# DillionLowry/NeuralCodecs

Hardware: AMD Instinct MI355X
Metric: audio-seconds/sec encode+decode (x real-time), DAC-44.1kHz B=32 (higher is better)
Workload: dtype f32; 1 GPU; DAC 44.1kHz 8kbps encode+decode, batch=32 x 1 s clips per GPU (BASELINE configs[1]); clips_per_gpu=32, global_batch=32, collective=none

## Files before the change

neuralcodecs_amd/csrc/nc_chunk.hip:

```cpp
#include <algorithm>

#include "nc_limits.h"
#include "nc_model.h"

namespace nc {

namespace {

int64_t ceil_div(int64_t a, int64_t b) { return (a + b - 1) / b; }
int64_t round_up(int64_t a, int64_t m) { return ceil_div(a, m) * m; }

void halo_from_layers(const int32_t* er, int ne, const int32_t* dr, int nd, int final_reach, int W, int vq_max, int64_t align, nc_halo* out) {
    if (ne <= 0 || ne > 8 || nd <= 0 || nd > 8) fail(NC_EINVAL, "encoder/decoder rate lists must hold 1..8 entries");
    int64_t l = final_reach, r = final_reach, hop = 1;
    if (W > 1) { l += W - 1; r += W - 1; }
    for (int i = ne - 1; i >= 0; --i) {
        const int64_t s = er[i], p = (s + 1) / 2;
        if (s <= 0) fail(NC_EINVAL, "encoder rate must be positive");
        l = l * s + p; r = r * s + (2 * s - 1 - p);
        l += 39; r += 39;
        hop *= s;
    }
    l += 3; r += 3;
    int64_t a = 3, b = 3, H = 1;
// ... 47 lines not shown
    if (setting < 0) return P;
    int64_t chunk = 0;
    if (setting > 0) chunk = round_up(setting, h.align);
    else if (!fits) chunk = auto_chunk(h, kind == CK_DECODE);
    if (chunk <= 0 || frames <= chunk) return P;
    P.chunk = chunk;
    P.n_chunks = ceil_div(frames, chunk);
    if (kind == CK_ENCODE) { P.halo_l = h.enc_right; P.halo_r = h.enc_left; }
    if (kind == CK_DECODE) { P.halo_l = h.dec_right; P.halo_r = h.dec_left; }
    return P;
}

struct Window { int64_t f0, f1, w0, w1; };
Window window_of(const ChunkPlan& P, int64_t j, int64_t frames) {
    Window w;
    w.f0 = j * P.chunk; w.f1 = std::min(frames, w.f0 + P.chunk);
    w.w0 = std::max<int64_t>(0, w.f0 - P.halo_l); w.w1 = std::min(frames, w.f1 + P.halo_r);
    return w;
}
int64_t max_window(const ChunkPlan& P, int64_t frames) { return std::min(frames, P.chunk + P.halo_l + P.halo_r); }

}

void Codec::copy2d(void* dst, bool dst_host, size_t dpitch, const void* src, bool src_host, size_t spitch, size_t width, size_t rows) {
    if (!width || !rows) return;
    if (!dst_host && !src_host) { launch_copy_rows(dst, dpitch, src, spitch, width, rows, stream); return; }
    const hipMemcpyKind kind = dst_host ? (src_host ? hipMemcpyHostToHost : hipMemcpyDeviceToHost) : hipMemcpyHostToDevice;
    if (rows == 1 || (width == dpitch && width == spitch)) NC_HIP(hipMemcpyAsync(dst, src, width * rows, kind, stream));
    else NC_HIP(hipMemcpy2DAsync(dst, dpitch, src, spitch, width, rows, kind, stream));
}

static void dac_halo(const nc_dac_config& c, nc_halo* out) {
    halo_from_layers(c.encoder_rates, c.n_encoder_rates, c.decoder_rates, c.n_decoder_rates, 1, 0, 1, 1, out);
}

ChunkPlan DacModel::chunk_plan(ChunkKind kind, int B, int64_t Tz) const {
    if (B <= 0 || Tz <= 0) fail(NC_EINVAL, "B and frames must be positive");
    nc_halo h{};
    dac_halo(cfg, &h);
    const bool fits = chunk_frames != 0 || oneshot_fits(cfg.encoder_rates, cfg.n_encoder_rates, cfg.encoder_dim, cfg.decoder_rates,
                                                        cfg.n_decoder_rates, cfg.decoder_dim, kind, Tz);
    ChunkPlan P = make_plan(chunk_frames, h, kind, Tz, fits);
    const int64_t W = P.n_chunks > 1 ? max_window(P, Tz) : Tz;
    int64_t maxel = 0;
    if (kind == CK_ENCODE) {
        int c = cfg.encoder_dim;
        int64_t L = W * hop;
        maxel = (int64_t)c * pitch16(L);
        for (int i = 0; i < cfg.n_encoder_rates; ++i) { c *= 2; L /= cfg.encoder_rates[i]; maxel = std::max(maxel, (int64_t)c * pitch16(L)); }
    } else if (kind == CK_DECODE) {
        int64_t L = W;
        maxel = (int64_t)cfg.decoder_dim * pitch16(L);
        for (int i = 0; i < cfg.n_decoder_rates; ++i) { L *= cfg.decoder_rates[i]; maxel = std::max(maxel, (int64_t)(cfg.decoder_dim >> (i + 1)) * pitch16(L)); }
    }
    P.arena_bytes = 3 * (int64_t)B * maxel * 4;
    return P;
}

void DacModel::encode_chunked(const ChunkPlan& P, bool host, const float* pcm, int B, int64_t T, int sample_rate, int n_q, int64_t* codes, float* z,
                              float* latents, int64_t* codes_tq) {
    if (!pcm || !(codes || codes_tq)) fail(NC_EINVAL, "pcm and codes must not be null");
    if (B <= 0 || T <= 0) fail(NC_EINVAL, "B and T must be positive");
    if (T > (int64_t)1 << 30) fail(NC_EINVAL, "clip too long");
    use_device();
    const int nq = codes_tq ? cfg.n_codebooks : ((n_q <= 0 || n_q > cfg.n_codebooks) ? cfg.n_codebooks : n_q);
    const int D = cfg.codebook_dim;
    const int64_t Tz = frames(T);
    for (int64_t j = 0; j < P.n_chunks; ++j) {
        const Window w = window_of(P, j, Tz);
        const int64_t s0 = w.w0 * hop, Tw = std::min(T, w.w1 * hop) - s0, Wf = w.w1 - w.w0, k0 = w.f0 - w.w0, n = w.f1 - w.f0;
        ck_in.reserve((size_t)B * Tw * 4);
        ck_codes.reserve((size_t)B * nq * Wf * 8);
        copy2d(ck_in.p, false, (size_t)Tw * 4, pcm + s0, host, (size_t)T * 4, (size_t)Tw * 4, (size_t)B);
        if (codes_tq) {
            encode_code_matrix_dev(ck_in.as<float>(), B, Tw, sample_rate, ck_codes.as<int64_t>());
            copy2d(codes_tq + w.f0 * nq, host, (size_t)Tz * nq * 8, ck_codes.as<int64_t>() + k0 * nq, false, (size_t)Wf * nq * 8, (size_t)n * nq * 8, (size_t)B);
            continue;
        }
        if (z) ck_a.reserve((size_t)B * latent * Wf * 4);
        if (latents) ck_b.reserve((size_t)B * nq * D * Wf * 4);
        encode_dev(ck_in.as<float>(), B, Tw, sample_rate, n_q, ck_codes.as<int64_t>(), z ? ck_a.as<float>() : nullptr, latents ? ck_b.as<float>() : nullptr);
        copy2d(codes + w.f0, host, (size_t)Tz * 8, ck_codes.as<int64_t>() + k0, false, (size_t)Wf * 8, (size_t)n * 8, (size_t)B * nq);
        if (z) copy2d(z + w.f0, host, (size_t)Tz * 4, ck_a.as<float>() + k0, false, (size_t)Wf * 4, (size_t)n * 4, (size_t)B * latent);
        if (latents) copy2d(latents + w.f0, host, (size_t)Tz * 4, ck_b.as<float>() + k0, false, (size_t)Wf * 4, (size_t)n * 4, (size_t)B * nq * D);
    }
}

void DacModel::from_codes_chunked(const ChunkPlan& P, bool host, const int64_t* codes, int B, int n_q, int64_t Tz, float* z) {
    if (!codes || !z) fail(NC_EINVAL, "codes and z must not be null");
    if (B <= 0 || Tz <= 0 || n_q <= 0 || n_q > cfg.n_codebooks) fail(NC_EINVAL, "bad codes shape [%d,%d,%lld]", B, n_q, (long long)Tz);
    use_device();
    for (int64_t j = 0; j < P.n_chunks; ++j) {
        const Window w = window_of(P, j, Tz);
        const int64_t n = w.f1 - w.f0;
        ck_codes.reserve((size_t)B * n_q * n * 8);
        ck_a.reserve((size_t)B * latent * n * 4);
        copy2d(ck_codes.p, false, (size_t)n * 8, codes + w.f0, host, (size_t)Tz * 8, (size_t)n * 8, (size_t)B * n_q);
        from_codes_dev(ck_codes.as<int64_t>(), B, n_q, n, ck_a.as<float>());
        copy2d(z + w.f0, host, (size_t)Tz * 4, ck_a.p, false, (size_t)n * 4, (size_t)n * 4, (size_t)B * latent);
    }
}

void DacModel::decode_chunked(const ChunkPlan& P, bool host, const float* z, const int64_t* codes_tq, int n_q, int B, int64_t Tz, float* pcm) {
    if (!(z || codes_tq) || !pcm) fail(NC_EINVAL, "z and pcm must not be null");
    if (B <= 0 || Tz <= 0) fail(NC_EINVAL, "B and frames must be positive");
    if (codes_tq && (n_q <= 0 || n_q > cfg.n_codebooks)) fail(NC_EINVAL, "bad code matrix shape [%d,%lld,%d]", B, (long long)Tz, n_q);
    use_device();
    int64_t H = 1;
    for (int i = 0; i < cfg.n_decoder_rates; ++i) H *= cfg.decoder_rates[i];
    const int64_t Lfull = decoded_len(Tz);
    for (int64_t j = 0; j < P.n_chunks; ++j) {
        const Window w = window_of(P, j, Tz);
        const int64_t Wf = w.w1 - w.w0, Lw = decoded_len(Wf), o0 = w.f0 * H, o1 = w.f1 == Tz ? Lfull : w.f1 * H, k0 = (w.f0 - w.w0) * H;
        if (o1 <= o0) continue;
        if (k0 + (o1 - o0) > Lw) fail(NC_ESTATE, "internal: decoded window of %lld samples does not cover its chunk", (long long)Lw);
        ck_out.reserve((size_t)B * Lw * 4);
        if (codes_tq) {
            ck_codes.reserve((size_t)B * Wf * n_q * 8);
            copy2d(ck_codes.p, false, (size_t)Wf * n_q * 8, codes_tq + w.w0 * n_q, host, (size_t)Tz * n_q * 8, (size_t)Wf * n_q * 8, (size_t)B);
            decode_code_matrix_dev(ck_codes.as<int64_t>(), B, Wf, n_q, ck_out.as<float>());
        } else {
            ck_a.reserve((size_t)B * latent * Wf * 4);
            copy2d(ck_a.p, false, (size_t)Wf * 4, z + w.w0, host, (size_t)Tz * 4, (size_t)Wf * 4, (size_t)B * latent);
            decode_dev(ck_a.as<float>(), B, Wf, ck_out.as<float>());
        }
        copy2d(pcm + o0, host, (size_t)Lfull * 4, ck_out.as<float>() + k0, false, (size_t)Lw * 4, (size_t)(o1 - o0) * 4, (size_t)B);
    }
}

static void snac_halo(const nc_snac_config& c, nc_halo* out) {
    if (c.n_vq_strides <= 0 || c.n_vq_strides > 8) fail(NC_EINVAL, "vq stride list must hold 1..8 entries");
    const int W = c.attn_window_size > 0 ? c.attn_window_size : 1;
    int64_t a = c.vq_strides[0], x = a, y = W;
    if (a <= 0) fail(NC_EINVAL, "vq stride must be positive");
    while (y) { const int64_t t = x % y; x = y; y = t; }
    const int64_t align = a / x * W;
    int vq_max = 1;
// ... 182 lines not shown
```

neuralcodecs_amd/csrc/nc_dac.hip:

```cpp
#include <cstdlib>
#include <cstring>

#include "nc_model.h"

namespace nc {

Codec::~Codec() {
    if (own_stream) (void)hipStreamDestroy(own_stream);
}

void Codec::init_device(int device_index) {
    int n = 0;
    if (hipGetDeviceCount(&n) != hipSuccess || n <= 0) fail(NC_EDEVICE, "no HIP device available (the engine has no CPU fallback)");
    if (device_index < 0 || device_index >= n) fail(NC_EINVAL, "device index %d out of range (0..%d)", device_index, n - 1);
    device = device_index;
    NC_HIP(hipSetDevice(device));
    hipDeviceProp_t prop;
    NC_HIP(hipGetDeviceProperties(&prop, device));
    if (std::strncmp(prop.gcnArchName, "gfx950", 6) != 0)
        fail(NC_EDEVICE, "device %d is %s; this engine is built for gfx950 (MI355X) only", device, prop.gcnArchName);
    cu_count = prop.multiProcessorCount;
    lds_per_cu = prop.maxSharedMemoryPerMultiProcessor;
    NC_HIP(hipStreamCreateWithFlags(&own_stream, hipStreamNonBlocking));
    stream = own_stream;
}

void Codec::use_device() const { NC_HIP(hipSetDevice(device)); }

void Codec::switch_stream(hipStream_t s) {
    if (s == stream) return;
    use_device();
    hipEvent_t e;
// ... 143 lines not shown
        load_alpha(b, p + ".block.0.alpha", in_dim, dec[bi].a_up);
        load_wn_conv(b, p + ".block.1", dec[bi].up, in_dim, out_dim, 2 * s, s, (s + 1) / 2, 1, true, NC_KC_CONV_UP);
        for (int u = 0; u < 3; ++u) {
            snprintf(nm, sizeof nm, "decoder.model.%d.block.%d", bi + 1, u + 2);
            const std::string q = nm;
            load_alpha(b, q + ".block.0.alpha", out_dim, dec[bi].ru[u].a1);
            load_wn_conv(b, q + ".block.1", dec[bi].ru[u].c7, out_dim, out_dim, 7, 1, 3 * kDil[u], kDil[u], false, NC_KC_CONV_K7);
            load_alpha(b, q + ".block.2.alpha", out_dim, dec[bi].ru[u].a2);
            load_wn_conv(b, q + ".block.3", dec[bi].ru[u].c1, out_dim, out_dim, 1, 1, 0, 1, false, NC_KC_CONV_K1);
        }
    }
    snprintf(nm, sizeof nm, "decoder.model.%d.alpha", cfg.n_decoder_rates + 1);
    load_alpha(b, nm, out_dim, dec_alpha_out);
    snprintf(nm, sizeof nm, "decoder.model.%d", cfg.n_decoder_rates + 2);
    load_wn_conv(b, nm, dec_out, out_dim, 1, 7, 1, 3, 1, false, NC_KC_HEAD);
    NC_HIP(hipDeviceSynchronize());
    loaded = true;
}

int64_t DacModel::decoded_len(int64_t fr) const {
    int64_t L = fr;
    for (int i = 0; i < cfg.n_decoder_rates; ++i) {
        const int s = cfg.decoder_rates[i];
        L = (L - 1) * s - 2 * ((s + 1) / 2) + 2 * s;
    }
    return L;
}

static int64_t row_pitch(int64_t L) {
    static const bool on = env_flag("NC_DAC_PITCH");
    return (on && L >= 256) ? ((L + 15) & ~(int64_t)15) : L;
}

float* DacModel::run_res_unit(ResUnit& ru, int dil, float* cur, int C, int64_t L, int B, int& cur_idx, const float* alpha_next) {
    (void)dil;
    const int64_t P = row_pitch(L);
    const int h_idx = (cur_idx + 1) % 3, o_idx = (cur_idx + 2) % 3;
    float* h = act[h_idx].as<float>();
    float* o = act[o_idx].as<float>();
    ConvIO io{};
    io.x = cur; io.x_bstride = (int64_t)C * P; io.x_cstride = P; io.x_len = (int32_t)L; io.Tin = L;
    io.alpha_in = ru.a1.as<float>(); io.alpha_out = ru.a2.as<float>();
    static const bool wide_192 = env_flag("NC_WIDE_FUSE_192");
    if (fuse_res_units && can_fuse_res_unit(ru.c7, ru.c1) && (C != 192 || wide_192)) {
        io.res = cur; io.fuse_k1 = &ru.c1; io.alpha_out2 = alpha_next;
        io.y = o; io.y_bstride = (int64_t)C * P; io.y_cstride = P;
        launch_conv(ru.c7, io, B, stream, &prof);
        cur_idx = o_idx;
        return o;
    }
    io.y = h; io.y_bstride = (int64_t)C * P; io.y_cstride = P;
    launch_conv(ru.c7, io, B, stream, &prof);
    ConvIO i2{};
    i2.x = h; i2.x_bstride = (int64_t)C * P; i2.x_cstride = P; i2.x_len = (int32_t)L; i2.Tin = L;
    i2.res = cur; i2.alpha_out = alpha_next;
    i2.y = o; i2.y_bstride = (int64_t)C * P; i2.y_cstride = P;
    launch_conv(ru.c1, i2, B, stream, &prof);
    cur_idx = o_idx;
    return o;
}

void DacModel::encode_dev(const float* pcm, int B, int64_t T, int sample_rate, int n_q, int64_t* codes, float* z, float* latents) {
    if (!loaded) fail(NC_ESTATE, "weights not loaded (call nc_codec_load_weights first)");
    if (!pcm || !codes) fail(NC_EINVAL, "pcm and codes must not be null");
    if (B <= 0 || T <= 0) fail(NC_EINVAL, "B and T must be positive");
    if (sample_rate != 0 && sample_rate != cfg.sample_rate)
        fail(NC_EINVAL, "Input audio sample rate %dHz does not match model sample rate %dHz", sample_rate, cfg.sample_rate);
    if (T > (int64_t)1 << 30) fail(NC_EINVAL, "clip too long");
    use_device();
    const int nq = (n_q <= 0 || n_q > cfg.n_codebooks) ? cfg.n_codebooks : n_q;
    const int64_t Tp = padded_len(T), Tz = frames(T);
    int64_t maxel = 0;
    {
        int c = cfg.encoder_dim;
        int64_t L = Tp;
        maxel = (int64_t)c * row_pitch(L);
        for (int i = 0; i < cfg.n_encoder_rates; ++i) {
            c *= 2;
            L /= cfg.encoder_rates[i];
            if ((int64_t)c * row_pitch(L) > maxel) maxel = (int64_t)c * row_pitch(L);
        }
    }
    for (auto& a : act) a.reserve((size_t)B * maxel * sizeof(float));
    const int D = cfg.codebook_dim;
    resid.reserve((size_t)B * latent * Tz * 4);
    zq.reserve((size_t)B * latent * Tz * 4);
    lat.reserve((size_t)B * nq * D * Tz * 4);
    st.reserve((size_t)B * D * Tz * 4);

    int C = cfg.encoder_dim;
    int64_t L = Tp;
    int cur_idx = 0;
    float* cur = act[0].as<float>();
    {
        ConvIO io{};
        io.x = pcm; io.x_bstride = T; io.x_cstride = T; io.x_len = (int32_t)T; io.Tin = Tp;
        io.y = cur; io.y_bstride = (int64_t)C * row_pitch(L); io.y_cstride = row_pitch(L);
        launch_conv(enc_stem, io, B, stream, &prof);
    }
    for (int bi = 0; bi < cfg.n_encoder_rates; ++bi) {
        for (int u = 0; u < 3; ++u)
            cur = run_res_unit(enc[bi].ru[u], kDil[u], cur, C, L, B, cur_idx, u == 2 ? enc[bi].a_down.as<float>() : nullptr);
        const int s = cfg.encoder_rates[bi];
        const int64_t Lo = enc[bi].down.out_len(L);
        const int o_idx = (cur_idx + 1) % 3;
        float* o = act[o_idx].as<float>();
        ConvIO io{};
        io.x = cur; io.x_bstride = (int64_t)C * row_pitch(L); io.x_cstride = row_pitch(L); io.x_len = (int32_t)L; io.Tin = L;
        if (bi + 1 == cfg.n_encoder_rates) io.alpha_out = enc_alpha_out.as<float>();
        io.y = o; io.y_bstride = (int64_t)2 * C * row_pitch(Lo); io.y_cstride = row_pitch(Lo);
        launch_conv(enc[bi].down, io, B, stream, &prof);
        (void)s;
        cur = o; cur_idx = o_idx; C *= 2; L = Lo;
    }
    if (L != Tz) fail(NC_ESTATE, "internal: encoder produced %lld frames, expected %lld", (long long)L, (long long)Tz);
    float* residual = resid.as<float>();
    {
        ConvIO io{};
        io.x = cur; io.x_bstride = (int64_t)C * row_pitch(L); io.x_cstride = row_pitch(L); io.x_len = (int32_t)L; io.Tin = L;
        io.y = residual; io.y_bstride = (int64_t)latent * Tz; io.y_cstride = Tz;
        launch_conv(enc_out, io, B, stream, &prof);
    }
    float* zq_d = z ? z : zq.as<float>();
    float* lat_d = latents ? latents : lat.as<float>();
    if (launch_dac_rvq_fused(rvq_stages.as<RvqStage>(), nq, latent, D, cfg.codebook_size, residual, B, Tz, codes, zq_d, lat_d, stream, &prof)) return;
    NC_HIP(hipMemsetAsync(zq_d, 0, (size_t)B * latent * Tz * 4, stream));
    for (int i = 0; i < nq; ++i) {
        ConvIO pi{};
        pi.x = residual; pi.x_bstride = (int64_t)latent * Tz; pi.x_cstride = Tz; pi.x_len = (int32_t)Tz; pi.Tin = Tz;
        pi.y = lat_d + (int64_t)i * D * Tz; pi.y_bstride = (int64_t)nq * D * Tz; pi.y_cstride = Tz;
        launch_conv(*in_proj[i], pi, B, stream, &prof);
        launch_vq_argmin(*codebooks[i], lat_d + (int64_t)i * D * Tz, (int64_t)nq * D * Tz, B, Tz, codes + (int64_t)i * Tz,
                         (int64_t)nq * Tz, st.as<float>(), stream, &prof);
        ConvIO po{};
        po.x = st.as<float>(); po.x_bstride = (int64_t)D * Tz; po.x_cstride = Tz; po.x_len = (int32_t)Tz; po.Tin = Tz;
        po.y = zq_d; po.y_bstride = (int64_t)latent * Tz; po.y_cstride = Tz;
        po.rvq_zq = zq_d; po.rvq_res = residual; po.epi = EPI_RVQ;
        launch_conv(*out_proj[i], po, B, stream, &prof);
    }
}

void DacModel::from_codes_dev(const int64_t* codes, int B, int n_q, int64_t Tz, float* z) {
    if (!loaded) fail(NC_ESTATE, "weights not loaded (call nc_codec_load_weights first)");
    if (!codes || !z) fail(NC_EINVAL, "codes and z must not be null");
    if (B <= 0 || Tz <= 0 || n_q <= 0 || n_q > cfg.n_codebooks) fail(NC_EINVAL, "bad codes shape [%d,%d,%lld]", B, n_q, (long long)Tz);
    use_device();
    const int D = cfg.codebook_dim;
    st.reserve((size_t)B * D * Tz * 4);
    NC_HIP(hipMemsetAsync(z, 0, (size_t)B * latent * Tz * 4, stream));
    for (int i = 0; i < n_q; ++i) {
        launch_vq_gather(*codebooks[i], codes + (int64_t)i * Tz, (int64_t)n_q * Tz, B, Tz, st.as<float>(), stream, &prof);
        ConvIO po{};
        po.x = st.as<float>(); po.x_bstride = (int64_t)D * Tz; po.x_cstride = Tz; po.x_len = (int32_t)Tz; po.Tin = Tz;
        po.y = z; po.y_bstride = (int64_t)latent * Tz; po.y_cstride = Tz;
        po.rvq_zq = z; po.rvq_res = nullptr; po.epi = EPI_RVQ;
        launch_conv(*out_proj[i], po, B, stream, &prof);
    }
}

__global__ void code_matrix_transpose_kernel(const int64_t* __restrict__ src, int64_t* __restrict__ dst, int B, int R, int C) {
    const int64_t i = (int64_t)blockIdx.x * 256 + threadIdx.x;
    if (i >= (int64_t)B * R * C) return;
    const int64_t c = i % C, r = (i / C) % R, b = i / ((int64_t)R * C);
    dst[(b * C + c) * R + r] = src[i];
}

void DacModel::decode_code_matrix_dev(const int64_t* codes_tq, int B, int64_t Tz, int n_q, float* pcm) {
    if (!codes_tq || !pcm) fail(NC_EINVAL, "codes and pcm must not be null");
    if (B <= 0 || Tz <= 0 || n_q <= 0 || n_q > cfg.n_codebooks) fail(NC_EINVAL, "bad code matrix shape [%d,%lld,%d]", B, (long long)Tz, n_q);
    use_device();
    codes_ws.reserve((size_t)B * n_q * Tz * 8);
    zq.reserve((size_t)B * latent * Tz * 4);
    const int64_t n = (int64_t)B * Tz * n_q;
    hipLaunchKernelGGL(code_matrix_transpose_kernel, dim3((unsigned)((n + 255) / 256)), dim3(256), 0, stream, codes_tq, codes_ws.as<int64_t>(), B, (int)Tz, n_q);
    NC_HIP(hipGetLastError());
    from_codes_dev(codes_ws.as<int64_t>(), B, n_q, Tz, zq.as<float>());
    decode_dev(zq.as<float>(), B, Tz, pcm);
}

void DacModel::encode_code_matrix_dev(const float* pcm, int B, int64_t T, int sample_rate, int64_t* codes_tq) {
    if (!pcm || !codes_tq) fail(NC_EINVAL, "pcm and codes must not be null");
    if (B <= 0 || T <= 0) fail(NC_EINVAL, "B and T must be positive");
    use_device();
    const int nq = cfg.n_codebooks;
    const int64_t Tz = frames(T);
    codes_ws.reserve((size_t)B * nq * Tz * 8);
    encode_dev(pcm, B, T, sample_rate, 0, codes_ws.as<int64_t>(), nullptr, nullptr);
    const int64_t n = (int64_t)B * Tz * nq;
    hipLaunchKernelGGL(code_matrix_transpose_kernel, dim3((unsigned)((n + 255) / 256)), dim3(256), 0, stream, codes_ws.as<int64_t>(), codes_tq, B, nq, (int)Tz);
    NC_HIP(hipGetLastError());
}

void DacModel::decode_dev(const float* z, int B, int64_t Tz, float* pcm) {
    if (!loaded) fail(NC_ESTATE, "weights not loaded (call nc_codec_load_weights first)");
    if (!z || !pcm) fail(NC_EINVAL, "z and pcm must not be null");
    if (B <= 0 || Tz <= 0) fail(NC_EINVAL, "B and frames must be positive");
    use_device();
    int64_t maxel = (int64_t)cfg.decoder_dim * row_pitch(Tz);
    {
        int64_t L = Tz;
        for (int i = 0; i < cfg.n_decoder_rates; ++i) {
            L = dec[i].up.out_len(L);
            const int64_t c = cfg.decoder_dim >> (i + 1);
            if (c * row_pitch(L) > maxel) maxel = c * row_pitch(L);
        }
    }
    for (auto& a : act) a.reserve((size_t)B * maxel * sizeof(float));
    int C = cfg.decoder_dim;
    int64_t L = Tz;
    int cur_idx = 0;
    float* cur = act[0].as<float>();
    {
        ConvIO io{};
        io.x = z; io.x_bstride = (int64_t)latent * Tz; io.x_cstride = Tz; io.x_len = (int32_t)Tz; io.Tin = Tz;
        io.alpha_out = dec[0].a_up.as<float>();
        io.y = cur; io.y_bstride = (int64_t)C * row_pitch(L); io.y_cstride = row_pitch(L);
        launch_conv(dec_in, io, B, stream, &prof);
    }
    for (int bi = 0; bi < cfg.n_decoder_rates; ++bi) {
        const int Co = C / 2;
        const int64_t Lo = dec[bi].up.out_len(L);
        const int o_idx = (cur_idx + 1) % 3;
        float* o = act[o_idx].as<float>();
        ConvIO io{};
        io.x = cur; io.x_bstride = (int64_t)C * row_pitch(L); io.x_cstride = row_pitch(L); io.x_len = (int32_t)L; io.Tin = L;
        io.y = o; io.y_bstride = (int64_t)Co * row_pitch(Lo); io.y_cstride = row_pitch(Lo);
        launch_conv(dec[bi].up, io, B, stream, &prof);
        cur = o; cur_idx = o_idx; C = Co; L = Lo;
        const float* a_next = bi + 1 < cfg.n_decoder_rates ? dec[bi + 1].a_up.as<float>() : dec_alpha_out.as<float>();
        for (int u = 0; u < 3; ++u) cur = run_res_unit(dec[bi].ru[u], kDil[u], cur, C, L, B, cur_idx, u == 2 ? a_next : nullptr);
    }
    {
        ConvIO io{};
        io.x = cur; io.x_bstride = (int64_t)C * row_pitch(L); io.x_cstride = row_pitch(L); io.x_len = (int32_t)L; io.Tin = L;
        io.y = pcm; io.y_bstride = L; io.y_cstride = L;
        io.epi = EPI_TANH;
        launch_conv(dec_out, io, B, stream, &prof);
    }
}

}
```

neuralcodecs_amd/csrc/nc_model.h:

```cpp
#pragma once
#include <memory>

#include "nc_common.h"
#include "nc_conv.h"
#include "nc_elem.h"

namespace nc {

const char* get_last_error();
void fold_weight_norm_dac(const float* v, const float* g, int64_t d0, int64_t inner, float* w);
void fold_weight_norm_snac(const float* v, const float* g, int64_t d0, int64_t inner, float* w);

struct Codebook {
    int N = 0, D = 0;
    DevBuf cbT;
    DevBuf cb;
    DevBuf c2;
    void build(const float* host_cb, int N, int D);
};
struct RvqStage {
    const float* w_inT;
    const float* b_in;
    const float* w_out;
    const float* b_out;
    const float* cbT;
    const float* c2;
    const float* cb;
};
bool launch_dac_rvq_fused(const RvqStage* stages_dev, int n_q, int L, int D, int N, const float* residual, int B, int64_t T, int64_t* codes,
                          float* zq, float* latents, hipStream_t s, Profiler* prof);
void launch_vq_argmin(const Codebook& cb, const float* z_e, int64_t ze_bstride, int B, int64_t T, int64_t* codes,
                      int64_t codes_bstride, float* st, hipStream_t s, Profiler* prof);
void op_euclid_rvq(const float* residual_in, int B, int D, int64_t T, const float* books_host, int n_q, int N, int form, int64_t* codes_host,
                   float* residual_out);
void launch_vq_gather(const Codebook& cb, const int64_t* codes, int64_t codes_bstride, int B, int64_t T, float* out, hipStream_t s,
                      Profiler* prof);

// ... 36 lines not shown
    nc_dac_config cfg{};
    int latent = 0, hop = 1;
    bool fuse_res_units = true;

    struct ResUnit {
        DevBuf a1, a2;
        ConvLayer c7, c1;
    };
    ConvLayer enc_stem;
    struct EncBlk {
        ResUnit ru[3];
        DevBuf a_down;
        ConvLayer down;
    } enc[8];
    DevBuf enc_alpha_out;
    ConvLayer enc_out;

    std::vector<std::unique_ptr<ConvLayer>> in_proj, out_proj;
    std::vector<std::unique_ptr<Codebook>> codebooks;
    std::vector<std::unique_ptr<DevBuf>> rvq_dense;
    DevBuf rvq_stages;

    ConvLayer dec_in;
    struct DecBlk {
        DevBuf a_up;
        ConvLayer up;
        ResUnit ru[3];
    } dec[8];
    DevBuf dec_alpha_out;
    ConvLayer dec_out;

    DevBuf act[3], resid, zq, lat, st, codes_ws, h_in, h_out, h_codes, h_aux0, h_aux1;

    explicit DacModel(const nc_dac_config& c);
    void load(const Blob& blob) override;
    int64_t padded_len(int64_t T) const { return (T + hop - 1) / hop * hop; }
    int64_t frames(int64_t T) const { return (T + hop - 1) / hop; }
    int64_t decoded_len(int64_t frames) const;
    void encode_dev(const float* pcm, int B, int64_t T, int sample_rate, int n_q, int64_t* codes, float* z, float* latents);
    void decode_dev(const float* z, int B, int64_t frames, float* pcm);
    void from_codes_dev(const int64_t* codes, int B, int n_q, int64_t frames, float* z);
    void decode_code_matrix_dev(const int64_t* codes_tq, int B, int64_t frames, int n_q, float* pcm);
    void encode_code_matrix_dev(const float* pcm, int B, int64_t T, int sample_rate, int64_t* codes_tq);
    ChunkPlan chunk_plan(ChunkKind kind, int B, int64_t frames) const;
    void encode_chunked(const ChunkPlan& P, bool host, const float* pcm, int B, int64_t T, int sample_rate, int n_q, int64_t* codes, float* z,
                        float* latents, int64_t* codes_tq);
    void decode_chunked(const ChunkPlan& P, bool host, const float* z, const int64_t* codes_tq, int n_q, int B, int64_t frames, float* pcm);
    void from_codes_chunked(const ChunkPlan& P, bool host, const int64_t* codes, int B, int n_q, int64_t frames, float* z);

  private:
    float* run_res_unit(ResUnit& ru, int dil, float* cur, int C, int64_t L, int B, int& cur_idx, const float* alpha_next);
};

struct SnacModel : Codec {
    nc_snac_config cfg{};
    int latent = 0, hop = 1;
    int64_t pad_to = 1;

    struct ResUnit {
        DevBuf a1, a2;
        DwConvLayer dw;
        ConvLayer c7;
        ConvLayer c1;
        SnacFusedUnit fu;
    };
    struct Mha {
        int C = 0;
        DevBuf gamma, beta, cs, sn;
        ConvLayer qkv, out;
    };
    ConvLayer enc_stem;
    struct EncBlk {
        ResUnit ru[3];
        DevBuf a_down;
        ConvLayer down;
    } enc[8];
    Mha enc_mha, dec_mha;
    DwConvLayer enc_out_dw, dec_in_dw;
    ConvLayer enc_out, dec_in;

    std::vector<std::unique_ptr<ConvLayer>> in_proj, out_proj;
    std::vector<std::unique_ptr<Codebook>> codebooks;

    struct DecBlk {
// ... 131 lines not shown
```

neuralcodecs_amd/csrc/nc_util.hip:

```cpp
#include <cmath>
#include <mutex>
#include <set>
#include <tuple>

#include "nc_common.h"
#include "nc_model.h"

namespace nc {

static thread_local std::string g_last_error;
void set_last_error(const char* msg) { g_last_error = msg ? msg : ""; }
const char* get_last_error() { return g_last_error.c_str(); }

namespace {
struct EnvRow { const char* name; char kind; const char* doc; };
const EnvRow kEnv[] = {
    {"NC_NO_FLAT", 'b', "one-clip column tiles instead of the flattened (clip, column) axis"},
    {"NC_NO_FLAT_GN", 'b', "one-clip tiles wherever GroupNorm sums are emitted"},
    {"NC_CO_GROUP", 'i', "cap of the row-tile groups (1 = one weight panel per XCD)"},
    {"NC_NO_WIDE_FUSE", 'b', "no whole-channel fused residual units (C = 256)"},
    {"NC_WIDE_FUSE_192", 'b', "whole-channel fused unit at C = 192 as well"},
    {"NC_NO_FUSE", 'b', "every residual unit in two launches"},
    {"NC_NO_TILE_ALTS", 'b', "primary row-tile height only"},
    {"NC_TM_PICK", 'i', "force a packed row-tile variant"},
// ... 3 lines not shown
    {"NC_NO_XR", 'b', "generic B-fragment addressing in the conv template (no constant-pitch immediate offsets)"},
    {"NC_NO_XV", 'b', "legacy instances with item-wise window staging everywhere (no XV-only instances)"},
    {"NC_XV_K7_MIN_COLS", 'i', "columns per clip from which the k = 7 convolutions take the XV-only instances (0: wherever the rows are 64-byte aligned)"},
    {"NC_NO_XV_K7", 'b', "legacy instances for the k = 7 residual-unit convolutions (no XV-only instances on the long rows)"},
    {"NC_NO_NARROW", 'b', "no 3-wave narrow variants"},
    {"NC_NO_SLIM", 'b', "no half-size reduction blocks for narrow long rows"},
    {"NC_NO_SUBPIXEL", 'b', "per-phase launches for power-of-two strided transposed convolutions"},
    {"NC_NO_SUBPIXEL_ANY", 'b', "per-phase launches for the other strides (3, 5)"},
    {"NC_NO_CONV1X1", 'b', "pointwise layers through the windowed template"},
    {"NC_NO_SKINNY", 'b', "no skinny projection kernel (Cout <= 16)"},
    {"NC_NO_THIN", 'b', "PCM heads through the matrix-core template"},
    {"NC_THIN_NO_VEC", 'p', "scalar window loads in the thin-output kernel"},
    {"NC_NO_THIN_INM", 'b', "summed copy + plain head instead of the input-mode head"},
    {"NC_NO_STEM", 'b', "stems through the matrix-core template"},
    {"NC_NO_TINY_TILES", 'b', "no smallest-tile rule for tiny grids"},
    {"NC_TINY_BLOCKS", 'i', "grid size below which the tiny-grid rule applies (256)"},
    {"NC_NO_DIST_SMALL", 'b', "segmented staging on small grids"},
    {"NC_DIST_MAX_GRID", 'i', "largest grid that takes distributed staging (768)"},
    {"NC_NO_CONV_SMALL", 'b', "no short-row 16x16x4 kernel"},
    {"NC_SMALL_MAX_GRID", 'i', "largest short-row grid (2048)"},
    {"NC_SMALL_WIDE_BELOW", 'i', "template grid below which the 32-column short-row form is taken (512)"},
    {"NC_SMALL_K1_COLS", 'i', "columns up to which k = 1 layers take the short-row kernel (4096; 0 = off)"},
    {"NC_SMALL_TN", 'i', "force the short-row column tiles (1 | 2 | 4)"},
    {"NC_SMALL_ROLLED", 'b', "rolled short-row loop"},
    {"NC_DAC_RVQ_STAGEWISE", 'p', "DAC quantizer stage by stage"},
    {"NC_EUCLID_NO_MFMA", 'p', "vector Euclidean codebook search"},
    {"NC_ENCODEC_NO_FUSE", 'b', "padded / activated copies instead of the fused SConv1d input mode"},
    {"NC_ENCODEC_NO_OVERLAP", 'b', "segment groups one after the other"},
    {"NC_NO_GN_FUSE", 'b', "stand-alone GroupNorm sums"},
    {"NC_NO_GN_FINISH", 'b', "separate GroupNorm final launch"},
    {"NC_NO_IN2", 'b', "summed copies instead of the two-input staging mode"},
    {"NC_NO_CONV3S", 'b', "windowed k = 3 instead of the streaming kernel"},
    {"NC_DAC_PITCH", 'b', "DAC activation rows at pitch L rounded up to 16 samples (64-byte aligned rows: the 696-step layers take the XV-only instances; measured slower)"},
    {"NC_NO_DOWN2", 'b', "Encodec 48 kHz encoder: the windowed two-input instance for the stride-2 down-convolution instead of the streaming kernel"},
    {"NC_NO_DOWN4", 'b', "Encodec 48 kHz encoder: summed copy + windowed instance for the stride-4 down-convolution instead of the streaming kernel"},
    {"NC_NO_DOWN5", 'b', "Encodec 48 kHz encoder: summed copy + windowed instance for the stride-5 down-convolution instead of the streaming kernel"},
    {"NC_NO_UP_PITCH", 'b', "Encodec transposed convolutions write dense rows (the trimmed view of the stride-5 layer then starts on an odd sample)"},
    {"NC_NO_UP4", 'b', "Encodec 48 kHz decoder: summed copy + windowed instance for the stride-4 up-convolution instead of the streaming kernel"},
    {"NC_NO_UP2", 'b', "Encodec 48 kHz decoder: the windowed two-input instance for the stride-2 up-convolution instead of the streaming kernel"},
    {"NC_RMS_TWO_PASS", 'b', "Encodec RMS scale as two launches (chunk sums, final) instead of the one-launch form"},
    {"NC_NO_RES_A", 'b', "residual blocks of the Encodec 48 kHz outer stages: shortcut and k = 3 branch as two launches instead of the fused first pass"},
    {"NC_SYNC_ACQUIRE", 'b', "agent-scope acquire fence behind the persistent LSTM's flag poll and in front of the in-launch GroupNorm finish"},
    {"NC_LSTM_STEPWISE", 'b', "one LSTM launch per step"},
    {"NC_LSTM_CHUNKS", 'i', "layer-pipeline chunks of the per-layer persistent LSTM (6; 1 = layers in sequence)"},
    {"NC_LSTM_EVEN_CHUNKS", 'b', "equal LSTM chunks"},
    {"NC_LSTM_UB", 'i', "hidden-unit blocks per LSTM workgroup (2 | 4)"},
    {"NC_LSTM_NO_HTILE", 'b', "persistent LSTM: every wavefront fetches its own h operands, W_hh in LDS (the form before the LDS h tile)"},
    {"NC_LSTM_NO_ELU", 'b', "the consumer applies the ELU behind an SLSTM"},
    {"NC_LSTM_FAKE_TIMEOUT", 'b', "tests: report the first persistent LSTM launch as timed out"},
    {"NC_SNAC_NO_FUSE", 'b', "SNAC residual units in two launches (depthwise, pointwise)"},
    {"NC_SNAC_FUSE_MIN_COLS", 'i', "columns (clips x steps) from which the one-launch SNAC residual unit is taken (65536)"},
    {"NC_SNAC_FUSE_MAX_ELEMS", 'i', "channels x steps of ONE clip up to which the one-launch SNAC residual unit is taken (2^30: its 32-bit lane offsets; tests lower it)"},
    {"NC_SNAC_UNIT_TRACE", 's', "file for the in-kernel stamps of the first one-launch SNAC residual unit at C = 96"},
    {"NC_DW_NO_VEC", 'b', "scalar depthwise kernel"},
    {"NC_LN_TILE", 'i', "LayerNorm tile width (8 | 16; 0 = one thread per column)"},
    {"NC_ATTN_NO_MFMA", 'b', "vector local-attention kernel"},
    {"NC_RCCL_LIB", 's', "the one RCCL library to open"},
    {"NC_LAUNCH_LOG", 's', "launch log for the per-class PMC attribution"},
    {"NC_CONV_TRACE_FILE", 's', "-DNC_CONV_TRACE builds: file for the in-kernel phase trace of the convolution template (tools/probe/conv_trace.py)"},
    {"NC_CONV_TRACE_SEL", 's', "-DNC_CONV_TRACE builds: \"K,Cin,dilation\" of the launch to trace (default 7,384,1)"},
};
const EnvRow& env_row(const char* name, char kind) {
    for (const EnvRow& r : kEnv)
        if (std::strcmp(r.name, name) == 0) {
            if (r.kind != kind) fail(NC_ESTATE, "switch %s is registered as kind '%c', read as '%c'", name, r.kind, kind);
            return r;
// ... 180 lines not shown
```

Baseline: 597.1 audio-seconds/sec.

## Split DAC one-shot batches into two halves on concurrent streams

DAC encode, decode and from-codes calls now split the batch into two halves and run each half on its own HIP stream, with fork/join events and an optional launch skew. Activation buffers are offset per half, so the two halves' kernels can overlap on the GPU and fill idle compute units left by small or tail-heavy grids. Chunked paths and profiling keep a single stream. The cost is twice the kernel launches at half the grid size each, plus possible contention between the halves.

```diff
diff --git a/neuralcodecs_amd/csrc/nc_chunk.hip b/neuralcodecs_amd/csrc/nc_chunk.hip
--- a/neuralcodecs_amd/csrc/nc_chunk.hip
+++ b/neuralcodecs_amd/csrc/nc_chunk.hip
@@ -103,6 +103,14 @@
 
 static void dac_halo(const nc_dac_config& c, nc_halo* out) {
     halo_from_layers(c.encoder_rates, c.n_encoder_rates, c.decoder_rates, c.n_decoder_rates, 1, 0, 1, 1, out);
+}
+
+namespace {
+struct SplitHold {
+    DacModel& m;
+    explicit SplitHold(DacModel& m_) : m(m_) { ++m.split_hold; }
+    ~SplitHold() { --m.split_hold; }
+};
 }
 
 ChunkPlan DacModel::chunk_plan(ChunkKind kind, int B, int64_t Tz) const {
@@ -131,6 +139,7 @@
 void DacModel::encode_chunked(const ChunkPlan& P, bool host, const float* pcm, int B, int64_t T, int sample_rate, int n_q, int64_t* codes, float* z,
                               float* latents, int64_t* codes_tq) {
     if (!pcm || !(codes || codes_tq)) fail(NC_EINVAL, "pcm and codes must not be null");
+    SplitHold one_stream(*this);
     if (B <= 0 || T <= 0) fail(NC_EINVAL, "B and T must be positive");
     if (T > (int64_t)1 << 30) fail(NC_EINVAL, "clip too long");
     use_device();
@@ -159,6 +168,7 @@
 
 void DacModel::from_codes_chunked(const ChunkPlan& P, bool host, const int64_t* codes, int B, int n_q, int64_t Tz, float* z) {
     if (!codes || !z) fail(NC_EINVAL, "codes and z must not be null");
+    SplitHold one_stream(*this);
     if (B <= 0 || Tz <= 0 || n_q <= 0 || n_q > cfg.n_codebooks) fail(NC_EINVAL, "bad codes shape [%d,%d,%lld]", B, n_q, (long long)Tz);
     use_device();
     for (int64_t j = 0; j < P.n_chunks; ++j) {
@@ -174,6 +184,7 @@
 
 void DacModel::decode_chunked(const ChunkPlan& P, bool host, const float* z, const int64_t* codes_tq, int n_q, int B, int64_t Tz, float* pcm) {
     if (!(z || codes_tq) || !pcm) fail(NC_EINVAL, "z and pcm must not be null");
+    SplitHold one_stream(*this);
     if (B <= 0 || Tz <= 0) fail(NC_EINVAL, "B and frames must be positive");
     if (codes_tq && (n_q <= 0 || n_q > cfg.n_codebooks)) fail(NC_EINVAL, "bad code matrix shape [%d,%lld,%d]", B, (long long)Tz, n_q);
     use_device();
diff --git a/neuralcodecs_amd/csrc/nc_dac.hip b/neuralcodecs_amd/csrc/nc_dac.hip
--- a/neuralcodecs_amd/csrc/nc_dac.hip
+++ b/neuralcodecs_amd/csrc/nc_dac.hip
@@ -1,3 +1,4 @@
+#include <algorithm>
 #include <cstdlib>
 #include <cstring>
 
@@ -207,12 +208,70 @@
     return (on && L >= 256) ? ((L + 15) & ~(int64_t)15) : L;
 }
 
-float* DacModel::run_res_unit(ResUnit& ru, int dil, float* cur, int C, int64_t L, int B, int& cur_idx, const float* alpha_next) {
+void DacModel::launched(Lane& ln) {
+    if (++ln.launches == ln.skew_at) NC_HIP(hipEventRecord(split_skew, ln.s));
+}
+
+void DacModel::reserve_act(int B, int64_t clip_elems) {
+    for (auto& a : act) a.reserve((size_t)B * clip_elems * sizeof(float) + 64);
+}
+
+static const int kSplitMinB = 8;
+
+template <class F>
+void DacModel::run_halves(int B, int64_t clip_elems, int skew_default, F&& body) {
+    static const bool off = env_flag("NC_DAC_NO_SPLIT");
+    static const long min_b = env_int("NC_DAC_SPLIT_MIN_B", kSplitMinB);
+    static const long force_b0 = env_int("NC_DAC_SPLIT_B0", 0);
+    static const long skew_env = env_int("NC_DAC_SPLIT_SKEW", -1);
+    Lane a;
+    a.s = stream; a.n = B;
+    const int B0 = (off || prof.on || split_hold > 0) ? 0 : dac_split_first_half(B, (int)min_b, (int)force_b0);
+    if (B0 == 0) {
+        body(a);
+        return;
+    }
+    if (!split_stream) {
+        NC_HIP(hipStreamCreateWithFlags(&split_stream, hipStreamNonBlocking));
+        NC_HIP(hipEventCreateWithFlags(&split_fork, hipEventDisableTiming));
+        NC_HIP(hipEventCreateWithFlags(&split_skew, hipEventDisableTiming));
+        NC_HIP(hipEventCreateWithFlags(&split_join, hipEventDisableTiming));
+    }
+    NC_HIP(hipEventRecord(split_fork, stream));
+    NC_HIP(hipStreamWaitEvent(split_stream, split_fork, 0));
+    try {
+        a.n = B0;
+        a.skew_at = skew_env >= 0 ? (int)std::min<long>(skew_env, 1 << 20) : skew_default;
+        body(a);
+        if (a.skew_at > 0) {
+            if (dac_split_skew(a.skew_at, a.launches) != a.skew_at)
+                NC_HIP(hipEventRecord(split_skew, stream));
+            NC_HIP(hipStreamWaitEvent(split_stream, split_skew, 0));
+        }
+        Lane b;
+        b.s = split_stream; b.b0 = B0; b.n = B - B0;
+        b.act_off = ((int64_t)B0 * clip_elems + 15) & ~(int64_t)15;
+        body(b);
+        NC_HIP(hipEventRecord(split_join, split_stream));
+        NC_HIP(hipStreamWaitEvent(stream, split_join, 0));
+    } catch (...) {
+        (void)hipStreamSynchronize(split_stream);
+        throw;
+    }
+}
+
+DacModel::~DacModel() {
+    if (split_stream) (void)hipStreamDestroy(split_stream);
+    for (hipEvent_t e : {split_fork, split_skew, split_join})
+        if (e) (void)hipEventDestroy(e);
+}
+
+float* DacModel::run_res_unit(ResUnit& ru, int dil, float* cur, int C, int64_t L, Lane& ln, int& cur_idx, const float* alpha_next) {
     (void)dil;
     const int64_t P = row_pitch(L);
     const int h_idx = (cur_idx + 1) % 3, o_idx = (cur_idx + 2) % 3;
-    float* h = act[h_idx].as<float>();
-    float* o = act[o_idx].as<float>();
+    float* h = act_at(ln, h_idx);
+    float* o = act_at(ln, o_idx);
     ConvIO io{};
     io.x = cur; io.x_bstride = (int64_t)C * P; io.x_cstride = P; io.x_len = (int32_t)L; io.Tin = L;
     io.alpha_in = ru.a1.as<float>(); io.alpha_out = ru.a2.as<float>();
@@ -220,17 +279,20 @@
     if (fuse_res_units && can_fuse_res_unit(ru.c7, ru.c1) && (C != 192 || wide_192)) {
         io.res = cur; io.fuse_k1 = &ru.c1; io.alpha_out2 = alpha_next;
         io.y = o; io.y_bstride = (int64_t)C * P; io.y_cstride = P;
-        launch_conv(ru.c7, io, B, stream, &prof);
+        launch_conv(ru.c7, io, ln.n, ln.s, &prof);
+        launched(ln);
         cur_idx = o_idx;
         return o;
     }
     io.y = h; io.y_bstride = (int64_t)C * P; io.y_cstride = P;
-    launch_conv(ru.c7, io, B, stream, &prof);
+    launch_conv(ru.c7, io, ln.n, ln.s, &prof);
+    launched(ln);
     ConvIO i2{};
     i2.x = h; i2.x_bstride = (int64_t)C * P; i2.x_cstride = P; i2.x_len = (int32_t)L; i2.Tin = L;
     i2.res = cur; i2.alpha_out = alpha_next;
     i2.y = o; i2.y_bstride = (int64_t)C * P; i2.y_cstride = P;
-    launch_conv(ru.c1, i2, B, stream, &prof);
+    launch_conv(ru.c1, i2, ln.n, ln.s, &prof);
+    launched(ln);
     cur_idx = o_idx;
     return o;
 }
@@ -256,62 +318,78 @@
             if ((int64_t)c * row_pitch(L) > maxel) maxel = (int64_t)c * row_pitch(L);
         }
     }
-    for (auto& a : act) a.reserve((size_t)B * maxel * sizeof(float));
+    reserve_act(B, maxel);
     const int D = cfg.codebook_dim;
     resid.reserve((size_t)B * latent * Tz * 4);
     zq.reserve((size_t)B * latent * Tz * 4);
     lat.reserve((size_t)B * nq * D * Tz * 4);
     st.reserve((size_t)B * D * Tz * 4);
-
+    run_halves(B, maxel, 0, [&](Lane& ln) { encode_lane(ln, pcm, T, nq, codes, z, latents); });
+}
+
+void DacModel::encode_lane(Lane& ln, const float* pcm, int64_t T, int nq, int64_t* codes, float* z, float* latents) {
+    const int B = ln.n, D = cfg.codebook_dim;
+    hipStream_t const stream = ln.s;
+    const int64_t Tp = padded_len(T), Tz = frames(T);
+    pcm += (int64_t)ln.b0 * T;
+    codes += (int64_t)ln.b0 * nq * Tz;
     int C = cfg.encoder_dim;
     int64_t L = Tp;
     int cur_idx = 0;
-    float* cur = act[0].as<float>();
+    float* cur = act_at(ln, 0);
     {
         ConvIO io{};
         io.x = pcm; io.x_bstride = T; io.x_cstride = T; io.x_len = (int32_t)T; io.Tin = Tp;
         io.y = cur; io.y_bstride = (int64_t)C * row_pitch(L); io.y_cstride = row_pitch(L);
         launch_conv(enc_stem, io, B, stream, &prof);
+        launched(ln);
     }
     for (int bi = 0; bi < cfg.n_encoder_rates; ++bi) {
         for (int u = 0; u < 3; ++u)
-            cur = run_res_unit(enc[bi].ru[u], kDil[u], cur, C, L, B, cur_idx, u == 2 ? enc[bi].a_down.as<float>() : nullptr);
-        const int s = cfg.encoder_rates[bi];
+            cur = run_res_unit(enc[bi].ru[u], kDil[u], cur, C, L, ln, cur_idx, u == 2 ? enc[bi].a_down.as<float>() : nullptr);
         const int64_t Lo = enc[bi].down.out_len(L);
         const int o_idx = (cur_idx + 1) % 3;
-        float* o = act[o_idx].as<float>();
+        float* o = act_at(ln, o_idx);
         ConvIO io{};
         io.x = cur; io.x_bstride = (int64_t)C * row_pitch(L); io.x_cstride = row_pitch(L); io.x_len = (int32_t)L; io.Tin = L;
         if (bi + 1 == cfg.n_encoder_rates) io.alpha_out = enc_alpha_out.as<float>();
         io.y = o; io.y_bstride = (int64_t)2 * C * row_pitch(Lo); io.y_cstride = row_pitch(Lo);
         launch_conv(enc[bi].down, io, B, stream, &prof);
-        (void)s;
+        launched(ln);
         cur = o; cur_idx = o_idx; C *= 2; L = Lo;
     }
     if (L != Tz) fail(NC_ESTATE, "internal: encoder produced %lld frames, expected %lld", (long long)L, (long long)Tz);
-    float* residual = resid.as<float>();
+    float* residual = resid.as<float>() + (int64_t)ln.b0 * latent * Tz;
     {
         ConvIO io{};
         io.x = cur; io.x_bstride = (int64_t)C * row_pitch(L); io.x_cstride = row_pitch(L); io.x_len = (int32_t)L; io.Tin = L;
         io.y = residual; io.y_bstride = (int64_t)latent * Tz; io.y_cstride = Tz;
         launch_conv(enc_out, io, B, stream, &prof);
-    }
-    float* zq_d = z ? z : zq.as<float>();
-    float* lat_d = latents ? latents : lat.as<float>();
-    if (launch_dac_rvq_fused(rvq_stages.as<RvqStage>(), nq, latent, D, cfg.codebook_size, residual, B, Tz, codes, zq_d, lat_d, stream, &prof)) return;
+        launched(ln);
+    }
+    float* zq_d = (z ? z : zq.as<float>()) + (int64_t)ln.b0 * latent * Tz;
+    float* lat_d = (latents ? latents : lat.as<float>()) + (int64_t)ln.b0 * nq * D * Tz;
+    float* st_d = st.as<float>() + (int64_t)ln.b0 * D * Tz;
+    if (launch_dac_rvq_fused(rvq_stages.as<RvqStage>(), nq, latent, D, cfg.codebook_size, residual, B, Tz, codes, zq_d, lat_d, stream, &prof)) {
+        launched(ln);
+        return;
+    }
     NC_HIP(hipMemsetAsync(zq_d, 0, (size_t)B * latent * Tz * 4, stream));
     for (int i = 0; i < nq; ++i) {
         ConvIO pi{};
         pi.x = residual; pi.x_bstride = (int64_t)latent * Tz; pi.x_cstride = Tz; pi.x_len = (int32_t)Tz; pi.Tin = Tz;
         pi.y = lat_d + (int64_t)i * D * Tz; pi.y_bstride = (int64_t)nq * D * Tz; pi.y_cstride = Tz;
         launch_conv(*in_proj[i], pi, B, stream, &prof);
+        launched(ln);
         launch_vq_argmin(*codebooks[i], lat_d + (int64_t)i * D * Tz, (int64_t)nq * D * Tz, B, Tz, codes + (int64_t)i * Tz,
-                         (int64_t)nq * Tz, st.as<float>(), stream, &prof);
+                         (int64_t)nq * Tz, st_d, stream, &prof);
+        launched(ln);
         ConvIO po{};
-        po.x = st.as<float>(); po.x_bstride = (int64_t)D * Tz; po.x_cstride = Tz; po.x_len = (int32_t)Tz; po.Tin = Tz;
+        po.x = st_d; po.x_bstride = (int64_t)D * Tz; po.x_cstride = Tz; po.x_len = (int32_t)Tz; po.Tin = Tz;
         po.y = zq_d; po.y_bstride = (int64_t)latent * Tz; po.y_cstride = Tz;
         po.rvq_zq = zq_d; po.rvq_res = residual; po.epi = EPI_RVQ;
         launch_conv(*out_proj[i], po, B, stream, &prof);
+        launched(ln);
     }
 }
 
@@ -320,16 +398,26 @@
     if (!codes || !z) fail(NC_EINVAL, "codes and z must not be null");
     if (B <= 0 || Tz <= 0 || n_q <= 0 || n_q > cfg.n_codebooks) fail(NC_EINVAL, "bad codes shape [%d,%d,%lld]", B, n_q, (long long)Tz);
     use_device();
-    const int D = cfg.codebook_dim;
-    st.reserve((size_t)B * D * Tz * 4);
+    st.reserve((size_t)B * cfg.codebook_dim * Tz * 4);
+    run_halves(B, 0, 0, [&](Lane& ln) { from_codes_lane(ln, codes, n_q, Tz, z); });
+}
+
+void DacModel::from_codes_lane(Lane& ln, const int64_t* codes, int n_q, int64_t Tz, float* z) {
+    const int B = ln.n, D = cfg.codebook_dim;
+    hipStream_t const stream = ln.s;
+    codes += (int64_t)ln.b0 * n_q * Tz;
+    z += (int64_t)ln.b0 * latent * Tz;
+    float* st_d = st.as<float>() + (int64_t)ln.b0 * D * Tz;
     NC_HIP(hipMemsetAsync(z, 0, (size_t)B * latent * Tz * 4, stream));
     for (int i = 0; i < n_q; ++i) {
-        launch_vq_gather(*codebooks[i], codes + (int64_t)i * Tz, (int64_t)n_q * Tz, B, Tz, st.as<float>(), stream, &prof);
+        launch_vq_gather(*codebooks[i], codes + (int64_t)i * Tz, (int64_t)n_q * Tz, B, Tz, st_d, stream, &prof);
+        launched(ln);
         ConvIO po{};
-        po.x = st.as<float>(); po.x_bstride = (int64_t)D * Tz; po.x_cstride = Tz; po.x_len = (int32_t)Tz; po.Tin = Tz;
+        po.x = st_d; po.x_bstride = (int64_t)D * Tz; po.x_cstride = Tz; po.x_len = (int32_t)Tz; po.Tin = Tz;
         po.y = z; po.y_bstride = (int64_t)latent * Tz; po.y_cstride = Tz;
         po.rvq_zq = z; po.rvq_res = nullptr; po.epi = EPI_RVQ;
         launch_conv(*out_proj[i], po, B, stream, &prof);
+        launched(ln);
     }
 }
 
@@ -380,30 +468,40 @@
             if (c * row_pitch(L) > maxel) maxel = c * row_pitch(L);
         }
     }
-    for (auto& a : act) a.reserve((size_t)B * maxel * sizeof(float));
+    reserve_act(B, maxel);
+    run_halves(B, maxel, 0, [&](Lane& ln) { decode_lane(ln, z, Tz, pcm); });
+}
+
+void DacModel::decode_lane(Lane& ln, const float* z, int64_t Tz, float* pcm) {
+    const int B = ln.n;
+    hipStream_t const stream = ln.s;
+    z += (int64_t)ln.b0 * latent * Tz;
+    pcm += (int64_t)ln.b0 * decoded_len(Tz);
     int C = cfg.decoder_dim;
     int64_t L = Tz;
     int cur_idx = 0;
-    float* cur = act[0].as<float>();
+    float* cur = act_at(ln, 0);
     {
         ConvIO io{};
         io.x = z; io.x_bstride = (int64_t)latent * Tz; io.x_cstride = Tz; io.x_len = (int32_t)Tz; io.Tin = Tz;
         io.alpha_out = dec[0].a_up.as<float>();
         io.y = cur; io.y_bstride = (int64_t)C * row_pitch(L); io.y_cstride = row_pitch(L);
         launch_conv(dec_in, io, B, stream, &prof);
+        launched(ln);
     }
     for (int bi = 0; bi < cfg.n_decoder_rates; ++bi) {
         const int Co = C / 2;
         const int64_t Lo = dec[bi].up.out_len(L);
         const int o_idx = (cur_idx + 1) % 3;
-        float* o = act[o_idx].as<float>();
+        float* o = act_at(ln, o_idx);
         ConvIO io{};
         io.x = cur; io.x_bstride = (int64_t)C * row_pitch(L); io.x_cstride = row_pitch(L); io.x_len = (int32_t)L; io.Tin = L;
         io.y = o; io.y_bstride = (int64_t)Co * row_pitch(Lo); io.y_cstride = row_pitch(Lo);
         launch_conv(dec[bi].up, io, B, stream, &prof);
+        launched(ln);
         cur = o; cur_idx = o_idx; C = Co; L = Lo;
         const float* a_next = bi + 1 < cfg.n_decoder_rates ? dec[bi + 1].a_up.as<float>() : dec_alpha_out.as<float>();
-        for (int u = 0; u < 3; ++u) cur = run_res_unit(dec[bi].ru[u], kDil[u], cur, C, L, B, cur_idx, u == 2 ? a_next : nullptr);
+        for (int u = 0; u < 3; ++u) cur = run_res_unit(dec[bi].ru[u], kDil[u], cur, C, L, ln, cur_idx, u == 2 ? a_next : nullptr);
     }
     {
         ConvIO io{};
@@ -411,7 +509,8 @@
         io.y = pcm; io.y_bstride = L; io.y_cstride = L;
         io.epi = EPI_TANH;
         launch_conv(dec_out, io, B, stream, &prof);
-    }
-}
-
-}
+        launched(ln);
+    }
+}
+
+}
diff --git a/neuralcodecs_amd/csrc/nc_dac_split.h b/neuralcodecs_amd/csrc/nc_dac_split.h
--- /dev/null
+++ b/neuralcodecs_amd/csrc/nc_dac_split.h
@@ -0,0 +1,13 @@
+#pragma once
+
+namespace nc {
+
+inline int dac_split_first_half(int B, int min_b, int b0) {
+    if (B < 2 || B < min_b) return 0;
+    if (b0 > 0) return b0 < B ? b0 : 0;
+    return (B + 1) / 2;
+}
+
+inline int dac_split_skew(int skew, int launches) { return skew < 0 ? 0 : (skew > launches ? launches : skew); }
+
+}
diff --git a/neuralcodecs_amd/csrc/nc_model.h b/neuralcodecs_amd/csrc/nc_model.h
--- a/neuralcodecs_amd/csrc/nc_model.h
+++ b/neuralcodecs_amd/csrc/nc_model.h
@@ -3,6 +3,7 @@
 
 #include "nc_common.h"
 #include "nc_conv.h"
+#include "nc_dac_split.h"
 #include "nc_elem.h"
 
 namespace nc {
@@ -105,7 +106,18 @@
 
     DevBuf act[3], resid, zq, lat, st, codes_ws, h_in, h_out, h_codes, h_aux0, h_aux1;
 
+    hipStream_t split_stream = nullptr;
+    hipEvent_t split_fork = nullptr, split_skew = nullptr, split_join = nullptr;
+    int split_hold = 0;
+    struct Lane {
+        hipStream_t s = nullptr;
+        int b0 = 0, n = 0;
+        int64_t act_off = 0;
+        int launches = 0, skew_at = 0;
+    };
+
     explicit DacModel(const nc_dac_config& c);
+    ~DacModel() override;
     void load(const Blob& blob) override;
     int64_t padded_len(int64_t T) const { return (T + hop - 1) / hop * hop; }
     int64_t frames(int64_t T) const { return (T + hop - 1) / hop; }
@@ -122,7 +134,15 @@
     void from_codes_chunked(const ChunkPlan& P, bool host, const int64_t* codes, int B, int n_q, int64_t frames, float* z);
 
   private:
-    float* run_res_unit(ResUnit& ru, int dil, float* cur, int C, int64_t L, int B, int& cur_idx, const float* alpha_next);
+    float* run_res_unit(ResUnit& ru, int dil, float* cur, int C, int64_t L, Lane& ln, int& cur_idx, const float* alpha_next);
+    float* act_at(const Lane& ln, int i) const { return act[i].as<float>() + ln.act_off; }
+    void launched(Lane& ln);
+    void reserve_act(int B, int64_t clip_elems);
+    template <class F>
+    void run_halves(int B, int64_t clip_elems, int skew_default, F&& body);
+    void encode_lane(Lane& ln, const float* pcm, int64_t T, int nq, int64_t* codes, float* z, float* latents);
+    void decode_lane(Lane& ln, const float* z, int64_t Tz, float* pcm);
+    void from_codes_lane(Lane& ln, const int64_t* codes, int n_q, int64_t Tz, float* z);
 };
 
 struct SnacModel : Codec {
diff --git a/neuralcodecs_amd/csrc/nc_util.hip b/neuralcodecs_amd/csrc/nc_util.hip
--- a/neuralcodecs_amd/csrc/nc_util.hip
+++ b/neuralcodecs_amd/csrc/nc_util.hip
@@ -59,6 +59,10 @@
     {"NC_NO_IN2", 'b', "summed copies instead of the two-input staging mode"},
     {"NC_NO_CONV3S", 'b', "windowed k = 3 instead of the streaming kernel"},
     {"NC_DAC_PITCH", 'b', "DAC activation rows at pitch L rounded up to 16 samples (64-byte aligned rows: the 696-step layers take the XV-only instances; measured slower)"},
+    {"NC_DAC_NO_SPLIT", 'b', "DAC one-shot calls on one stream (no half-batch split over the handle's side stream)"},
+    {"NC_DAC_SPLIT_MIN_B", 'i', "smallest batch whose DAC one-shot calls run as two half-batches on two streams (8)"},
+    {"NC_DAC_SPLIT_B0", 'i', "clips in the first half of a split DAC call (0 = even halves, the odd clip in the first)"},
+    {"NC_DAC_SPLIT_SKEW", 'i', "launches of head start the first half of a split DAC call gets (0 = both halves start together; clamped to the half's launches)"},
     {"NC_NO_DOWN2", 'b', "Encodec 48 kHz encoder: the windowed two-input instance for the stride-2 down-convolution instead of the streaming kernel"},
     {"NC_NO_DOWN4", 'b', "Encodec 48 kHz encoder: summed copy + windowed instance for the stride-4 down-convolution instead of the streaming kernel"},
     {"NC_NO_DOWN5", 'b', "Encodec 48 kHz encoder: summed copy + windowed instance for the stride-5 down-convolution instead of the streaming kernel"},
```

Measured after the change: 602.4 audio-seconds/sec (median of 6 runs). About the same (+0.9%).
